# isarandi/metro-pose3d

Hardware: AMD Instinct MI355X
Metric: crops/sec (256x256, RN50 stride16) (higher is better)
Workload: dtype f16

## Files before the change

### include/metro_hip.h

```cpp
#ifndef METRO_HIP_H
#define METRO_HIP_H

#include <stddef.h>
#include <stdint.h>

#ifdef __cplusplus
extern "C" {
#endif

#define METRO_ABI_VERSION 8

typedef enum MetroStatus {
    METRO_OK = 0,
    METRO_ERR_INVALID_ARG = -1,
    METRO_ERR_UNSUPPORTED = -2,
    METRO_ERR_HIP = -3,
    METRO_ERR_STATE = -4,
    METRO_ERR_NONFINITE = -5
} MetroStatus;

typedef enum MetroPrecision { METRO_PREC_F16 = 0, METRO_PREC_F32 = 1, METRO_PREC_F64 = 2, METRO_PREC_F32M = 3 } MetroPrecision;

typedef enum MetroDType { METRO_F16 = 0, METRO_F32 = 1, METRO_F64 = 2 } MetroDType;

// ... 92 lines not shown
    int32_t h_out, w_out, c_out;
    int32_t kh, kw, stride, dilation;
    int32_t pad_top, pad_left;
    int32_t has_prologue;
    int32_t relu;
    int32_t has_residual;
    int32_t res_h, res_w;
    int32_t res_stride, res_offset;
    int32_t out_dtype;
    int32_t in_dtype;
} MetroConvDesc;

int  metro_conv_f16(const MetroConvDesc* d, const void* d_in, const void* d_w, const float* d_bias,
                    const void* d_pro_scale, const void* d_pro_shift, const void* d_residual,
                    void* d_out, void* stream);
int  metro_conv_f16_pair(const MetroConvDesc* d, const void* d_in, const void* d_w, const float* d_bias,
                         const void* d_pro_scale, const void* d_pro_shift, void* d_out, int32_t split,
                         void* d_out2, void* stream);
int  metro_conv_f16_next(const MetroConvDesc* d, const void* d_in, const void* d_w, const float* d_bias,
                         const void* d_residual, void* d_out, const void* d_w2, const float* d_bias2,
                         const void* d_scale2, const void* d_shift2, void* d_out2, int32_t c2, void* stream);
int  metro_conv_f16_conv1_conv2(const MetroConvDesc* d, const void* d_x, const void* d_w1, const float* d_bias1, const void* d_pro_scale,
                                const void* d_pro_shift, const void* d_w2, const float* d_bias2, void* d_out, void* stream);
int  metro_conv_f16_next_proj(const MetroConvDesc* d, const void* d_in, const void* d_w, const float* d_bias, const void* d_x,
                              const void* d_w_sc, const float* d_bias_sc, const void* d_pro_scale, const void* d_pro_shift, void* d_out,
                              const void* d_w2, const float* d_bias2, const void* d_scale2, const void* d_shift2, void* d_out2,
                              int32_t c2, void* stream);
int  metro_conv_f16_next_rebuild(const MetroConvDesc* d, const void* d_in, const void* d_w, const float* d_bias, const void* d_x,
                                 const void* d_w_sc, const float* d_bias_sc, const void* d_pro_scale, const void* d_pro_shift,
                                 const void* d_t2_prev, const void* d_w3_prev, const float* d_bias3_prev, void* d_out, void* d_out_sub,
                                 int32_t sub_off, const void* d_w2, const float* d_bias2, const void* d_scale2, const void* d_shift2,
                                 void* d_out2, int32_t c2, void* stream);
int  metro_conv_b1_form(int32_t classic);
int  metro_conv_f16_gemm4w(const MetroConvDesc* d, const void* d_in, const void* d_w, const float* d_bias,
                           const void* d_pro_scale, const void* d_pro_shift, const void* d_residual, void* d_out,
                           int32_t split, void* d_out2, void* stream);
int  metro_stem_pool_f16(const void* d_prepped, const void* d_w, const float* d_bias, void* d_out, int32_t n,
                         int32_t side, void* stream);
int  metro_stem_pool_f32in(const float* d_images, const void* d_w, const float* d_bias, void* d_out, int32_t n,
                           int32_t side, void* stream);
int  metro_stem_pool_u8in(const uint8_t* d_images, const void* d_w, const float* d_bias, void* d_out, int32_t n,
                          int32_t side, void* stream);
int  metro_conv_f64acc(const MetroConvDesc* d, const void* d_in, const double* d_w,
                       const double* d_bias, const double* d_pro_scale,
                       const double* d_pro_shift, const void* d_residual, void* d_out,
                       void* stream);

int  metro_conv_f32m(const MetroConvDesc* d, const void* d_in, const float* d_w, const float* d_bias, const float* d_pro_scale,
                     const float* d_pro_shift, const void* d_residual, void* d_out, void* stream);

int  metro_prep_input_f16(const float* d_images, int32_t n, int32_t side, void* d_out, void* stream);
int  metro_images_u8_to_f32(const uint8_t* d_in, int64_t count, float* d_out, void* stream);

int  metro_warp_crop_u8(const uint8_t* d_image, int32_t h, int32_t w, int32_t row_stride,
                        const float* d_homographies, int32_t n, int32_t side, float* d_out, void* stream);

#define METRO_MAX_FRAMES 64
#define METRO_WARP_HOMOGRAPHY 0
#define METRO_WARP_DISTORTED 1
typedef struct MetroFrame {
    const uint8_t* data;
    int32_t h, w, row_stride;
    int32_t reserved;
} MetroFrame;
typedef struct MetroCropWarp {
    int32_t frame;
// ... 217 lines not shown
```

### metro_pose3d_amd/_lib.py

```python
from __future__ import annotations

import ctypes as C
import os

HERE = os.path.dirname(os.path.abspath(__file__))
LIB_PATH = os.environ.get('METRO_HIP_LIB') or os.path.join(HERE, 'libmetro_hip.so')

METRO_MAX_JOINTS = 64
ABI_VERSION = 8
METRO_PREC_F16, METRO_PREC_F32, METRO_PREC_F64, METRO_PREC_F32M = 0, 1, 2, 3
METRO_F16, METRO_F32, METRO_F64 = 0, 1, 2
PARAM_CONV_W, PARAM_BIAS, PARAM_PRO_SCALE, PARAM_PRO_SHIFT = 0, 1, 2, 3
LAYER_PREP, LAYER_CONV, LAYER_POOL, LAYER_SOFTARGMAX = 0, 1, 2, 3
FUSED_CONV1_IN_FRONT, FUSED_PROJECTION_SHORTCUT = 1, 2
FUSED_OUT_ON_CHIP, FUSED_REBUILT_SHORTCUT, FUSED_COMPACT_SHORTCUT = 4, 8, 16


class MetroSpec(C.Structure):
    _fields_ = [('arch', C.c_int32), ('stride', C.c_int32), ('n_joints_head', C.c_int32),
                ('depth', C.c_int32), ('centered_stride', C.c_int32), ('proc_side', C.c_int32),
                ('box_size_mm', C.c_float), ('base_width', C.c_int32), ('precision', C.c_int32),
                ('n_joints_out', C.c_int32), ('permutation', C.c_int32 * METRO_MAX_JOINTS)]


# ... 91 lines not shown
class MetroView(C.Structure):
    _fields_ = [('cos_roll', C.c_double), ('sin_roll', C.c_double), ('zoom', C.c_double), ('flip', C.c_int32),
                ('reserved', C.c_int32)]


_P = C.c_void_p
SIGNATURES = {
    'metro_plan_create': (C.c_int, [C.POINTER(MetroSpec), C.c_int32, C.POINTER(_P)]),
    'metro_plan_destroy': (C.c_int, [_P]),
    'metro_plan_workspace_bytes': (C.c_int64, [_P]),
    'metro_plan_param_bytes': (C.c_int64, [_P]),
    'metro_plan_num_params': (C.c_int32, [_P]),
    'metro_plan_param_info': (C.c_int, [_P, C.c_int32, C.POINTER(MetroParamInfo)]),
    'metro_plan_num_layers': (C.c_int32, [_P]),
    'metro_plan_layer_info': (C.c_int, [_P, C.c_int32, C.POINTER(MetroLayerInfo)]),
    'metro_plan_flops_per_image': (C.c_double, [_P]),
    'metro_plan_bind_params': (C.c_int, [_P, _P]),
    'metro_plan_layer_kernel': (C.c_int, [_P, C.c_int32, C.c_int32, C.c_char_p, C.c_int32]),
    'metro_kernel_notes': (C.c_int, [C.c_int32]),
    'metro_last_kernel_id': (C.c_char_p, []),
    'metro_plan_set_graph_max_batch': (C.c_int, [_P, C.c_int32]),
    'metro_forward': (C.c_int, [_P, _P, C.c_int32, _P, _P, _P]),
    'metro_forward_coords01': (C.c_int, [_P, _P, C.c_int32, _P, _P, _P, _P]),
    'metro_forward_u8': (C.c_int, [_P, _P, C.c_int32, _P, _P, _P, _P]),
    'metro_forward_status': (C.c_int, [_P, _P, C.c_int32, _P, C.POINTER(C.c_int32)]),
    'metro_plan_status_offset': (C.c_int64, [_P]),
    'metro_forward_upto': (C.c_int, [_P, _P, C.c_int32, _P, _P, _P, C.c_int32]),
    'metro_forward_timed': (C.c_int, [_P, _P, C.c_int32, _P, _P, _P, C.POINTER(C.c_float)]),
    'metro_conv_f16': (C.c_int, [C.POINTER(MetroConvDesc), _P, _P, _P, _P, _P, _P, _P, _P]),
    'metro_conv_f32m': (C.c_int, [C.POINTER(MetroConvDesc), _P, _P, _P, _P, _P, _P, _P, _P]),
    'metro_conv_f64acc': (C.c_int, [C.POINTER(MetroConvDesc), _P, _P, _P, _P, _P, _P, _P, _P]),
    'metro_conv_f16_pair': (C.c_int, [C.POINTER(MetroConvDesc), _P, _P, _P, _P, _P, _P, C.c_int32, _P, _P]),
    'metro_conv_b1_form': (C.c_int, [C.c_int32]),
    'metro_conv_f16_gemm4w': (C.c_int, [C.POINTER(MetroConvDesc), _P, _P, _P, _P, _P, _P, _P, C.c_int32, _P, _P]),
    'metro_conv_f16_conv1_conv2': (C.c_int, [C.POINTER(MetroConvDesc), _P, _P, _P, _P, _P, _P, _P, _P, _P]),
    'metro_conv_f16_next_proj': (C.c_int, [C.POINTER(MetroConvDesc)] + [_P] * 14 + [C.c_int32, _P]),
    'metro_conv_f16_next_rebuild': (C.c_int, [C.POINTER(MetroConvDesc)] + [_P] * 13 + [C.c_int32] + [_P] * 5 + [C.c_int32, _P]),
    'metro_conv_f16_next': (C.c_int, [C.POINTER(MetroConvDesc), _P, _P, _P, _P, _P, _P, _P, _P, _P, _P, C.c_int32, _P]),
    'metro_stem_pool_f16': (C.c_int, [_P, _P, _P, _P, C.c_int32, C.c_int32, _P]),
    'metro_stem_pool_f32in': (C.c_int, [_P, _P, _P, _P, C.c_int32, C.c_int32, _P]),
    'metro_stem_pool_u8in': (C.c_int, [_P, _P, _P, _P, C.c_int32, C.c_int32, _P]),
    'metro_prep_input_f16': (C.c_int, [_P, C.c_int32, C.c_int32, _P, _P]),
    'metro_images_u8_to_f32': (C.c_int, [_P, C.c_int64, _P, _P]),
    'metro_warp_crop_u8': (C.c_int, [_P, C.c_int32, C.c_int32, C.c_int32, _P, C.c_int32, C.c_int32, _P, _P]),
    'metro_warp_crops_frames_u8': (C.c_int, [C.POINTER(MetroFrame), C.c_int32, _P, C.c_int32, C.c_int32, _P, _P]),
    'metro_warp_crops_frames_planes': (C.c_int, [C.POINTER(MetroFramePlanes), C.c_int32, _P, C.c_int32, C.c_int32, _P,
                                                 _P]),
    'metro_warp_crops_frames_u8_to_u8': (C.c_int, [C.POINTER(MetroFrame), C.c_int32, _P, C.c_int32, C.c_int32, _P, _P]),
    'metro_warp_crops_frames_planes_to_u8': (C.c_int, [C.POINTER(MetroFramePlanes), C.c_int32, _P, C.c_int32, C.c_int32, _P,
                                                       _P]),
    'metro_eval_metrics': (C.c_int, [_P, _P, _P, C.c_int32, C.c_int32, C.c_float, _P, _P, _P, _P]),
    'metro_maxpool3x3s2_zeropad': (C.c_int, [_P, _P, C.c_int32, C.c_int32, C.c_int32, C.c_int32,
                                             C.c_int32, _P]),
    'metro_softargmax_scratch_bytes': (C.c_int64, [C.c_int32, C.c_int32, C.c_int32]),
    'metro_softargmax01': (C.c_int, [_P, C.c_int32, C.POINTER(MetroSpec), C.c_int32, _P, _P, _P]),
    'metro_backproject_bone_lengths': (C.c_int, [_P, _P, _P, C.c_int32, _P, C.c_int32, C.c_int32, C.POINTER(MetroSpec),
                                                 C.c_int32, C.c_int32, _P, _P, _P]),
    'metro_backproject_root_depth': (C.c_int, [_P, _P, _P, C.c_int32, C.POINTER(MetroSpec), C.c_int32, C.c_int32, _P, _P]),
    'metro_to_orig_cam': (C.c_int, [_P, _P, _P, _P, C.c_int32, C.c_int32, _P]),
    'metro_place_poses': (C.c_int, [_P, _P, _P, C.c_int32, C.POINTER(MetroSpec), C.c_int32, _P, C.c_int32, _P, _P, C.c_int32,
                                    _P, C.c_int32, _P, _P, _P, _P]),
    'metro_expand_views': (C.c_int, [_P, C.c_int32, C.POINTER(MetroView), C.c_int32, C.c_int32, _P, _P, _P]),
    'metro_look_at_boxes': (C.c_int, [_P, _P, C.c_int32, C.c_int32, _P, C.c_int32, C.c_int32, _P, _P, _P]),
    'metro_merge_views': (C.c_int, [_P, _P, _P, _P, _P, C.c_int32, C.c_int32, C.c_int32, _P, _P, _P, _P, _P]),
    'metro_heatmap_to_25d': (C.c_int, [_P, C.c_int32, C.POINTER(MetroSpec), _P, _P]),
    'metro_head_f16_scratch_bytes': (C.c_int64, [C.c_int32, C.c_int32, C.c_int32]),
# ... 98 lines not shown
```

### metro_pose3d_amd/csrc/conv3x3_c64.hip

```cpp
#ifndef METRO_WT_STORES
#define METRO_WT_STORES 1
#endif
#include "metro_common.h"
#include "gfx950_prims.h"

namespace metro {

namespace c64 {
constexpr int C = 64, TN = 128, NW = 8, NT = 512;
constexpr int W_BYTES = 9 * C * 128;
constexpr int SLAB_ROWS = 256;
constexpr int SLAB_BYTES = SLAB_ROWS * 128;
constexpr int SI = SLAB_BYTES / 1024 / NW;
constexpr int WI = W_BYTES / 1024 / NW;
constexpr int W_OFF = 0;
constexpr int SLAB_OFF = W_BYTES;
constexpr int ZERO_OFF = SLAB_OFF + 2 * SLAB_BYTES;
constexpr int OUT_OFF = ZERO_OFF + 256;
constexpr int OUT_ROW = C * 2 + 16;
constexpr int LDS_BYTES = OUT_OFF + TN * OUT_ROW;
constexpr int STORES = TN * (C / 8) / NT;
static_assert(LDS_BYTES <= 160 * 1024 && ZERO_OFF % 256 == 0, "LDS budget / zero-area alignment");
}

struct C64Args {
    const half_t* in;
    const half_t* w;
    const float* bias;
    half_t* out;
    int m_total, h, w_map, relu, n_tiles, tiles_per_block;
    const half_t* w1;
    const float* bias1;
    const half_t* pro_scale;
    const half_t* pro_shift;
    half_t* t1_dump;
};

template <bool PRE1>
__global__ __launch_bounds__(c64::NT) void conv3x3_c64_kernel(C64Args a) {
    using namespace c64;
    extern __shared__ __attribute__((aligned(16))) char smem[];
    const int tid = threadIdx.x;
    const int lane = tid & 63;
    const int wave = __builtin_amdgcn_readfirstlane(tid >> 6);
    const int wm = wave >> 2, wn = wave & 3;
    const int frag_row = lane & 31, frag_half = lane >> 5;
    const int t_begin = blockIdx.x * a.tiles_per_block;
    int t_end = t_begin + a.tiles_per_block;
    if (t_end > a.n_tiles) t_end = a.n_tiles;
    if (t_begin >= t_end) return;
    const half_t* zero = reinterpret_cast<const half_t*>(g_zero_page);
    const unsigned smem_base = lds_offset_of(smem);
    const int halo = a.w_map;
    const int hw = a.h * a.w_map;

    if (tid < 16) reinterpret_cast<uint4*>(smem + ZERO_OFF)[tid] = make_uint4(0, 0, 0, 0);

    const int lrow = lane >> 3, lch = lane & 7;
#pragma unroll
    for (int i = 0; i < WI; ++i) {
        const int grp = i * NW + wave;
        const int tap = grp >> 3, row = (grp & 7) * 8 + lrow;
        const half_t* src = a.w + (size_t)row * (9 * C) + tap * C + ((lch ^ swz<64>(row)) * 8);
        dma16(src, __builtin_amdgcn_readfirstlane(smem_base + W_OFF + grp * 1024));
    }
    auto issue_slab = [&](int tile, int buf) {
        const int m0 = tile * TN;
#pragma unroll
        for (int i = 0; i < SI; ++i) {
            const int srow = (i * NW + wave) * 8 + lrow;
            const int g = m0 - halo + srow;
            const bool ok = g >= 0 && g < a.m_total && srow < TN + 2 * halo;
            const half_t* src = ok ? a.in + (size_t)g * C + ((lch ^ swz<64>(srow)) * 8) : zero;
            dma16(src, __builtin_amdgcn_readfirstlane(smem_base + SLAB_OFF + buf * SLAB_BYTES + (i * NW + wave) * 1024));
        }
    };
    issue_slab(t_begin, 0);

    const int arow = wm * 32 + frag_row;
    const int a_base = W_OFF + arow * 128 + ((frag_half ^ swz<64>(arow)) << 4);
    float bias_v[4][4];
#pragma unroll
    for (int q = 0; q < 4; ++q) {
        const floatx4 bv = *reinterpret_cast<const floatx4*>(a.bias + wm * 32 + 8 * q + 4 * frag_half);
#pragma unroll
        for (int e = 0; e < 4; ++e) bias_v[q][e] = bv[e];
    }
    half8_t w1f[2][4], ps1[4], pb1[4];
    float bias1_v[2][4][4];
    if constexpr (PRE1) {
#pragma unroll
        for (int i = 0; i < 2; ++i) {
#pragma unroll
            for (int kk = 0; kk < 4; ++kk)
                w1f[i][kk] = *reinterpret_cast<const half8_t*>(a.w1 + (size_t)(i * 32 + frag_row) * C + kk * 16 + frag_half * 8);
#pragma unroll
            for (int q = 0; q < 4; ++q) {
                const floatx4 bv = *reinterpret_cast<const floatx4*>(a.bias1 + i * 32 + 8 * q + 4 * frag_half);
#pragma unroll
                for (int e = 0; e < 4; ++e) bias1_v[i][q][e] = bv[e];
            }
        }
#pragma unroll
        for (int kk = 0; kk < 4; ++kk) {
            ps1[kk] = *reinterpret_cast<const half8_t*>(a.pro_scale + kk * 16 + frag_half * 8);
            pb1[kk] = *reinterpret_cast<const half8_t*>(a.pro_shift + kk * 16 + frag_half * 8);
        }
    }
    wait_vm_and_barrier<0>();

    for (int t = t_begin; t < t_end; ++t) {
        const int buf = (t - t_begin) & 1;
        if (t != t_begin) {
            asm volatile("s_waitcnt vmcnt(%0)\n\ts_barrier" ::"n"(STORES) : "memory");
        }
        if (t + 1 < t_end) issue_slab(t + 1, buf ^ 1);

        if constexpr (PRE1) {
            char* sp = smem + SLAB_OFF + buf * SLAB_BYTES;
            const int srow = wave * 32 + frag_row;
            const int r_base = srow * 128 + ((frag_half ^ swz<64>(srow)) << 4);
            floatx16 a1[2];
#pragma unroll
            for (int e = 0; e < 16; ++e) { a1[0][e] = 0.f; a1[1][e] = 0.f; }
#pragma unroll
            for (int kk = 0; kk < 4; ++kk) {
                half8_t bf = *reinterpret_cast<const half8_t*>(sp + (r_base ^ (kk << 5)));
                bf = relu(bf * ps1[kk] + pb1[kk]);
                a1[0] = __builtin_amdgcn_mfma_f32_32x32x16_f16(w1f[0][kk], bf, a1[0], 0, 0, 0);
                a1[1] = __builtin_amdgcn_mfma_f32_32x32x16_f16(w1f[1][kk], bf, a1[1], 0, 0, 0);
            }
#pragma unroll
            for (int i = 0; i < 2; ++i)
#pragma unroll
                for (int q = 0; q < 4; ++q) {
                    half4_t hv;
#pragma unroll
                    for (int e = 0; e < 4; ++e) hv[e] = (half_t)relu(a1[i][4 * q + e] + bias1_v[i][q][e]);
                    *reinterpret_cast<half4_t*>(sp + srow * 128 + ((((4 * i + q) ^ swz<64>(srow)) << 4) | (frag_half << 3))) = hv;
                    if (a.t1_dump != nullptr && srow >= halo && srow < halo + TN)
                        *reinterpret_cast<half4_t*>(a.t1_dump + (size_t)(t * TN + srow - halo) * C + i * 32 + 8 * q + 4 * frag_half) = hv;
                }
            wait_lgkm_and_barrier();
        }
        const int m0 = t * TN;
        const int tl = wn * 32 + frag_row;
        const int rem = (m0 + tl) % hw;
        const int py = rem / a.w_map, px = rem - py * a.w_map;
        floatx16 acc;
#pragma unroll
        for (int e = 0; e < 16; ++e) acc[e] = 0.f;
        const int sl = SLAB_OFF + buf * SLAB_BYTES;
#pragma unroll
        for (int tap = 0; tap < 9; ++tap) {
            const int dr = tap / 3 - 1, ds = tap % 3 - 1;
            const bool ok = (unsigned)(py + dr) < (unsigned)a.h && (unsigned)(px + ds) < (unsigned)a.w_map;
            const int srow = halo + tl + dr * a.w_map + ds;
            const int b_base = ok ? sl + srow * 128 + ((frag_half ^ swz<64>(srow)) << 4) : ZERO_OFF;
#pragma unroll
            for (int kk = 0; kk < 4; ++kk) {
                const half8_t af = *reinterpret_cast<const half8_t*>(smem + tap * 8192 + (a_base ^ (kk << 5)));
                const half8_t bf = *reinterpret_cast<const half8_t*>(smem + (b_base ^ (kk << 5)));
                acc = __builtin_amdgcn_mfma_f32_32x32x16_f16(af, bf, acc, 0, 0, 0);
            }
        }
        char* ol = smem + OUT_OFF;
#pragma unroll
        for (int q = 0; q < 4; ++q) {
            half4_t hv;
#pragma unroll
            for (int e = 0; e < 4; ++e) {
                float v = acc[4 * q + e] + bias_v[q][e];
                if (a.relu) v = relu(v);
                hv[e] = (half_t)v;
            }
            *reinterpret_cast<half4_t*>(ol + tl * OUT_ROW + (wm * 32 + 8 * q + 4 * frag_half) * 2) = hv;
        }
        wait_lgkm_and_barrier();
#pragma unroll
        for (int r = 0; r < STORES; ++r) {
            const int idx = tid + r * NT;
            const int prow = idx >> 3, ch = idx & 7;
            const uint4 v = *reinterpret_cast<const uint4*>(ol + prow * OUT_ROW + ch * 16);
            store_out16(a.out + (size_t)(m0 + prow) * C + ch * 8, v);
        }
    }
}

bool conv3x3_c64_supported(const MetroConvDesc& d) {
    static const int enabled = tuning_knob("METRO_CONV_C64", 1);
    if (!enabled) return false;
    if (!(d.kh == 3 && d.kw == 3 && d.stride == 1 && d.dilation == 1 && d.pad_top == 1 && d.pad_left == 1 &&
          d.h_in == d.h_out && d.w_in == d.w_out && d.c_in == 64 && d.c_out == 64 && d.in_pix_stride == 64 &&
          !d.has_prologue && !d.has_residual && d.in_dtype == METRO_F16 && d.out_dtype == METRO_F16))
        return false;
    const long m = (long)d.n * d.h_out * d.w_out;
    return d.w_out <= 64 && c64::TN % d.w_out == 0 && (d.h_out * d.w_out) % c64::TN == 0 && m >= 4 * c64::TN;
}

int launch_conv3x3_c64(const MetroConvDesc& d, const void* in, const void* w, const float* bias, void* out, hipStream_t stream,
                       const ConvPre1* pre1) {
    if (!conv3x3_c64_supported(d)) { set_error("conv3x3_c64: unsupported layer"); return METRO_ERR_UNSUPPORTED; }
    const bool p1 = pre1 != nullptr && pre1->w1 != nullptr;
    if (note_kernel(p1 ? "conv3x3_c64<pre1>" : "conv3x3_c64")) return METRO_OK;
    C64Args a;
    a.in = static_cast<const half_t*>(in); a.w = static_cast<const half_t*>(w); a.bias = bias; a.out = static_cast<half_t*>(out);
    a.m_total = d.n * d.h_out * d.w_out; a.h = d.h_out; a.w_map = d.w_out; a.relu = d.relu;
    a.n_tiles = a.m_total / c64::TN;
    a.w1 = p1 ? static_cast<const half_t*>(pre1->w1) : nullptr; a.bias1 = p1 ? pre1->bias1 : nullptr;
    a.pro_scale = p1 ? static_cast<const half_t*>(pre1->pro_scale) : nullptr;
    a.pro_shift = p1 ? static_cast<const half_t*>(pre1->pro_shift) : nullptr;
    a.t1_dump = p1 ? static_cast<half_t*>(pre1->t1_dump) : nullptr;
    auto kern = p1 ? conv3x3_c64_kernel<true> : conv3x3_c64_kernel<false>;
    static PerDeviceInt cap[2];
    int grid_cap = 0;
    if (const int st = ensure_dyn_lds_and_grid_cap(reinterpret_cast<const void*>(kern), c64::NT, c64::LDS_BYTES, cap[p1 ? 1 : 0],
                                                   "conv3x3_c64", 1, &grid_cap))
        return st;
    a.tiles_per_block = (a.n_tiles + grid_cap - 1) / grid_cap;
    const int grid = (a.n_tiles + a.tiles_per_block - 1) / a.tiles_per_block;
    hipLaunchKernelGGL(kern, dim3(grid), dim3(c64::NT), c64::LDS_BYTES, stream, a);
    return launch_status("conv3x3_c64");
}

}
```

### metro_pose3d_amd/csrc/entries.cpp

```cpp
#include <cmath>
#include <cstring>

#include "metro_common.h"

namespace metro {

static thread_local char g_err[512] = "";

void set_error(const char* fmt, ...) {
    va_list ap;
    va_start(ap, fmt);
    vsnprintf(g_err, sizeof(g_err), fmt, ap);
    va_end(ap);
}
const char* get_error() { return g_err; }

static thread_local KernelNotes g_notes = {0, ""};
KernelNotes& kernel_notes() { return g_notes; }
bool note_kernel(const char* fmt, ...) {
    if (g_notes.mode == 0) return false;
    const size_t cap = sizeof(g_notes.ids) - 5;
    const size_t used = strlen(g_notes.ids);
    if (used >= 4 && strcmp(g_notes.ids + used - 4, " ...") == 0) return g_notes.mode == 2;
    char one[512];
// ... 65 lines not shown
                           static_cast<hipStream_t>(stream));
}

int metro_conv_f16_pair(const MetroConvDesc* d, const void* d_in, const void* d_w, const float* d_bias,
                        const void* d_pro_scale, const void* d_pro_shift, void* d_out, int32_t split,
                        void* d_out2, void* stream) {
    int st = validate_conv_desc(d);
    if (st) return st;
    METRO_CHECK_ARG(d_in && d_w && d_bias && d_out && d_out2 && d_pro_scale && d_pro_shift, "conv_f16_pair: NULL tensor pointer");
    ConvFused f;
    f.form = ConvForm::Pair;
    f.pair = {split, d->c_out - split, 1, d_out2};
    METRO_CHECK_ARG(conv_form_supported(*d, f), "conv_f16_pair: fp16 1x1 stride-1 convolution with prologue, without residual / ReLU on the "
                    "first output, c_in %% 64; split %d of c_out %d (split %% 256, rest %% 8)", split, d->c_out);
    return launch_conv_f16_dma(*d, d_in, d_w, d_bias, d_pro_scale, d_pro_shift, nullptr, d_out, static_cast<hipStream_t>(stream), f);
}

int metro_conv_f16_next(const MetroConvDesc* d, const void* d_in, const void* d_w, const float* d_bias,
                        const void* d_residual, void* d_out, const void* d_w2, const float* d_bias2,
                        const void* d_scale2, const void* d_shift2, void* d_out2, int32_t c2, void* stream) {
    int st = validate_conv_desc(d);
    if (st) return st;
    METRO_CHECK_ARG(d_in && d_w && d_bias && d_out && d_w2 && d_bias2 && d_scale2 && d_shift2 && d_out2,
                    "conv_f16_next: NULL tensor pointer");
    METRO_CHECK_ARG(!d->has_residual || d_residual, "conv_f16_next: residual tensor missing");
    ConvFused f;
    f.form = ConvForm::Next;
    f.next = {d_w2, d_bias2, d_scale2, d_shift2, d_out2, c2};
    METRO_CHECK_ARG(conv_form_supported(*d, f),
                    "conv_f16_next: built for 1x1 stride-1 64 -> 256 with c2 = 64 (block1) and 128 -> 512 with c2 = 128 (block2), fp16");
    return launch_conv_f16_dma(*d, d_in, d_w, d_bias, nullptr, nullptr, d_residual, d_out, static_cast<hipStream_t>(stream), f);
}

int metro_conv_f16_conv1_conv2(const MetroConvDesc* d, const void* d_x, const void* d_w1, const float* d_bias1, const void* d_pro_scale,
                               const void* d_pro_shift, const void* d_w2, const float* d_bias2, void* d_out, void* stream) {
    int st = validate_conv_desc(d);
    if (st) return st;
    METRO_CHECK_ARG(d_x && d_w1 && d_bias1 && d_pro_scale && d_pro_shift && d_w2 && d_bias2 && d_out, "conv_f16_conv1_conv2: NULL tensor pointer");
    METRO_CHECK_ARG(conv3x3_c64_supported(*d), "conv_f16_conv1_conv2: built for 3x3 stride-1 SAME 64 -> 64 on maps of <= 64 columns that tile into "
                    "128-pixel row pairs (block1 of the 256-pixel nets)");
    ConvPre1 p1;
    p1.w1 = d_w1; p1.bias1 = d_bias1; p1.pro_scale = d_pro_scale; p1.pro_shift = d_pro_shift;
    return launch_conv3x3_c64(*d, d_x, d_w2, d_bias2, d_out, static_cast<hipStream_t>(stream), &p1);
}

int metro_conv_f16_next_proj(const MetroConvDesc* d, const void* d_in, const void* d_w, const float* d_bias, const void* d_x,
                             const void* d_w_sc, const float* d_bias_sc, const void* d_pro_scale, const void* d_pro_shift, void* d_out,
                             const void* d_w2, const float* d_bias2, const void* d_scale2, const void* d_shift2, void* d_out2,
                             int32_t c2, void* stream) {
    int st = validate_conv_desc(d);
    if (st) return st;
    METRO_CHECK_ARG(d_in && d_w && d_bias && d_x && d_w_sc && d_bias_sc && d_pro_scale && d_pro_shift && d_w2 && d_bias2 &&
                        d_scale2 && d_shift2 && d_out2, "conv_f16_next_proj: NULL tensor pointer");
    ConvFused f;
    f.form = ConvForm::NextProj;
    f.next = {d_w2, d_bias2, d_scale2, d_shift2, d_out2, c2};
    f.psc = {d_x, d_w_sc, d_bias_sc, d_pro_scale, d_pro_shift};
    f.rb.out_mode = d_out == nullptr ? 1 : 0;
    METRO_CHECK_ARG(conv_form_supported(*d, f), "conv_f16_next_proj: built for 1x1 stride-1 64 -> 256 without prologue / residual, "
                    "c2 = 64 (block1/unit_1), fp16");
    return launch_conv_f16_dma(*d, d_in, d_w, d_bias, nullptr, nullptr, nullptr, d_out, static_cast<hipStream_t>(stream), f);
}

int metro_conv_f16_next_rebuild(const MetroConvDesc* d, const void* d_in, const void* d_w, const float* d_bias, const void* d_x,
                                const void* d_w_sc, const float* d_bias_sc, const void* d_pro_scale, const void* d_pro_shift,
                                const void* d_t2_prev, const void* d_w3_prev, const float* d_bias3_prev, void* d_out, void* d_out_sub,
                                int32_t sub_off, const void* d_w2, const float* d_bias2, const void* d_scale2, const void* d_shift2,
                                void* d_out2, int32_t c2, void* stream) {
    int st = validate_conv_desc(d);
    if (st) return st;
    METRO_CHECK_ARG(d_in && d_w && d_bias && d_x && d_w_sc && d_bias_sc && d_pro_scale && d_pro_shift && d_t2_prev && d_w3_prev && d_bias3_prev &&
                        d_w2 && d_bias2 && d_scale2 && d_shift2 && d_out2, "conv_f16_next_rebuild: NULL tensor pointer");
    METRO_CHECK_ARG((d_out != nullptr) != (d_out_sub != nullptr), "conv_f16_next_rebuild: exactly one of d_out (the whole sum) and d_out_sub (its "
                    "sub-sampled compact copy) must be given");
    METRO_CHECK_ARG(sub_off == 0 || sub_off == 1, "conv_f16_next_rebuild: sub_off %d must be 0 or 1", sub_off);
    ConvFused f;
    f.form = ConvForm::NextRebuild;
    f.next = {d_w2, d_bias2, d_scale2, d_shift2, d_out2, c2};
    f.psc = {d_x, d_w_sc, d_bias_sc, d_pro_scale, d_pro_shift};
    ConvRebuild& rb = f.rb;
    rb.t2_prev = d_t2_prev; rb.w3_prev = d_w3_prev; rb.bias3_prev = d_bias3_prev;
    if (d_out_sub != nullptr) {
        rb.out_mode = 2; rb.out_sub = d_out_sub; rb.sub_off = sub_off;
        rb.h_sub = (d->h_out - sub_off + 1) / 2; rb.w_sub = (d->w_out - sub_off + 1) / 2;
    }
    METRO_CHECK_ARG(conv_form_supported(*d, f), "conv_f16_next_rebuild: built for 1x1 stride-1 64 -> 256 without prologue / residual on maps "
                    "whose width is a power of two >= 16 and whose pixel count is a multiple of 64, c2 = 64 (block1/unit_2), fp16");
    return launch_conv_f16_dma(*d, d_in, d_w, d_bias, nullptr, nullptr, nullptr, d_out, static_cast<hipStream_t>(stream), f);
}

int metro_conv_b1_form(int32_t classic) {
    METRO_CHECK_ARG(classic == 0 || classic == 1, "metro_conv_b1_form: 0 (default dispatch) or 1 (classic single-role kernel)");
    conv_b1_set_form(classic);
    return METRO_OK;
}

int metro_conv_f16_gemm4w(const MetroConvDesc* d, const void* d_in, const void* d_w, const float* d_bias,
                          const void* d_pro_scale, const void* d_pro_shift, const void* d_residual, void* d_out,
                          int32_t split, void* d_out2, void* stream) {
    int st = validate_conv_desc(d);
    if (st) return st;
    METRO_CHECK_ARG(d_in && d_w && d_bias && d_out, "conv_f16_gemm4w: NULL tensor pointer");
    METRO_CHECK_ARG(!d->has_prologue || (d_pro_scale && d_pro_shift), "conv_f16_gemm4w: prologue tensors missing");
    METRO_CHECK_ARG(!d->has_residual || d_residual, "conv_f16_gemm4w: residual tensor missing");
    METRO_CHECK_ARG(split >= 0 && split < d->c_out && (split == 0 || d_out2), "conv_f16_gemm4w: bad split %d / missing second output", split);
    ConvSplit sp;
    sp.split = split; sp.c_out2 = d->c_out - split; sp.relu2 = 1; sp.out2 = d_out2;
    return launch_conv_gemm4w(*d, d_in, d_w, d_bias, d_pro_scale, d_pro_shift, d_residual, d_out,
                              static_cast<hipStream_t>(stream), split > 0 ? &sp : nullptr);
}

int metro_stem_pool_f16(const void* d_prepped, const void* d_w, const float* d_bias, void* d_out, int32_t n,
                        int32_t side, void* stream) {
    METRO_CHECK_ARG(d_prepped && d_w && d_bias && d_out, "stem_pool_f16: NULL tensor pointer");
    METRO_CHECK_ARG(n > 0, "stem_pool_f16: n = %d", n);
    METRO_CHECK_ARG(stem_pool_f16_supported(side, 64), "stem_pool_f16: side %d must be a multiple of 32 (and METRO_STEM_POOL != 0)", side);
    return launch_stem_pool_f16(d_prepped, d_w, d_bias, d_out, n, side, static_cast<hipStream_t>(stream));
}

int metro_stem_pool_f32in(const float* d_images, const void* d_w, const float* d_bias, void* d_out, int32_t n,
                          int32_t side, void* stream) {
    METRO_CHECK_ARG(d_images && d_w && d_bias && d_out, "stem_pool_f32in: NULL tensor pointer");
    METRO_CHECK_ARG(n > 0, "stem_pool_f32in: n = %d", n);
    METRO_CHECK_ARG(stem_pool_f32in_supported(side, 64), "stem_pool_f32in: side %d must be a multiple of 32 (and METRO_STEM_POOL / METRO_STEM_RAW != 0)", side);
    return launch_stem_pool_f32in(d_images, d_w, d_bias, d_out, n, side, static_cast<hipStream_t>(stream));
}
// ... 588 lines not shown
```

### metro_pose3d_amd/csrc/metro_common.h

```cpp
#pragma once
#include <hip/hip_runtime.h>
#include <cstdarg>
#include <cstdint>
#include <cstdio>
#include <cstdlib>

#include "../../include/metro_hip.h"

namespace metro {

void set_error(const char* fmt, ...);
const char* get_error();

#define METRO_CHECK_ARG(cond, ...)                  \
    do {                                            \
        if (!(cond)) {                              \
            ::metro::set_error(__VA_ARGS__);        \
            return METRO_ERR_INVALID_ARG;           \
        }                                           \
    } while (0)

#define METRO_HIP_CHECK(expr)                                                              \
    do {                                                                                   \
        hipError_t _e = (expr);                                                            \
// ... 219 lines not shown
                    const void* pro_scale, const void* pro_shift, const void* residual, void* out,
                    hipStream_t stream);
bool conv_f16_dma_supported(const MetroConvDesc& d);
int launch_conv_f16_dma(const MetroConvDesc& d, const void* in, const void* w, const float* bias,
                        const void* pro_scale, const void* pro_shift, const void* residual, void* out,
                        hipStream_t stream, const ConvFused& f = ConvFused{});
bool conv_form_supported(const MetroConvDesc& d, const ConvFused& f);
bool conv_f16_fuse2_supported(const MetroConvDesc& d, int c2);
bool conv_gemm4w_shape_ok(const MetroConvDesc& d, const ConvSplit* split);
bool conv_gemm4w_supported(const MetroConvDesc& d, const ConvSplit* split);
int launch_conv_gemm4w(const MetroConvDesc& d, const void* in, const void* w, const float* bias, const void* pro_scale,
                       const void* pro_shift, const void* residual, void* out, hipStream_t stream, const ConvSplit* split);
bool conv_pw64_supported(const MetroConvDesc& d, const ConvFused& f);
int launch_conv_pw64(const MetroConvDesc& d, const void* in, const void* w, const float* bias, const void* pro_scale,
                     const void* pro_shift, const void* residual, void* out, hipStream_t stream, const ConvFused& f);
bool conv_b1_chain_preferred();
void conv_b1_set_form(int classic);
bool classic_forms_forced();
bool conv_pws_supported(const MetroConvDesc& d);
int launch_conv_pws(const MetroConvDesc& d, const void* in, const void* w, const float* bias, const void* res, void* out, hipStream_t stream);
int launch_conv_b1_chain(const MetroConvDesc& d, const void* in, const void* w, const float* bias, void* out, hipStream_t stream,
                         const ConvFused& f);
bool stem_pool_f16_supported(int side, int base_width);
int launch_stem_pool_f16(const void* prepped, const void* w, const float* bias, void* out, int n, int side,
                         hipStream_t stream);
bool stem_pool_f32in_supported(int side, int base_width);
int launch_stem_pool_f32in(const float* images, const void* w, const float* bias, void* out, int n, int side,
                           hipStream_t stream);
int launch_stem_pool_u8in(const unsigned char* images, const void* w, const float* bias, void* out, int n, int side,
                          hipStream_t stream);
bool conv3x3_c64_supported(const MetroConvDesc& d);
int launch_conv3x3_c64(const MetroConvDesc& d, const void* in, const void* w, const float* bias, void* out, hipStream_t stream,
                       const ConvPre1* pre1 = nullptr);
bool conv3x3_slab_supported(const MetroConvDesc& d);
int launch_conv3x3_slab(const MetroConvDesc& d, const void* in, const void* w, const float* bias, void* out,
                        hipStream_t stream);
int launch_conv_f64acc(const MetroConvDesc& d, const void* in, const double* w, const double* bias,
                       const double* pro_scale, const double* pro_shift, const void* residual,
                       void* out, hipStream_t stream);
int launch_conv_f32m(const MetroConvDesc& d, const void* in, const float* w, const float* bias, const float* pro_scale,
                     const float* pro_shift, const void* residual, void* out, hipStream_t stream);
int launch_prep_input_f16(const float* images, int n, int side, void* out, hipStream_t stream);
int launch_prep_input_u8_f16(const unsigned char* images, int n, int side, void* out, hipStream_t stream);
int launch_images_u8_to_f32(const unsigned char* in, long count, float* out, hipStream_t stream);
struct FrameTable { MetroFrame f[METRO_MAX_FRAMES]; };
template <typename OutT>
int launch_warp_crops_frames_u8(const FrameTable& frames, int n_frames, const MetroCropWarp* crops, int n, int side,
                                OutT* out, hipStream_t stream);
struct FramePlanesTable { MetroFramePlanes f[METRO_MAX_FRAMES]; };
template <typename OutT>
int launch_warp_crops_frames_planes(const FramePlanesTable& frames, int n_frames, const MetroCropWarp* crops, int n,
                                    int side, OutT* out, hipStream_t stream);
template <typename OutT>
int launch_warp_crop_u8(const unsigned char* img, int h, int w, int row_stride, const float* homs, OutT* out,
                        int n, int side, hipStream_t stream);
int launch_eval_metrics(const float* pred, const float* truth, const unsigned char* valid, int n, int nj,
                        float threshold, float* dist, float* dist_pa, double* sums, hipStream_t stream);
int launch_maxpool(const void* in, void* out, int n, int h_in, int w_in, int c, int dtype,
                   hipStream_t stream);

struct SoftArgmaxArgs {
    int n, side, depth, n_joints_head, n_joints_out;
    int lrc, half_off;
    float box_size_mm;
    int proc_side;
    int perm[METRO_MAX_JOINTS];
// ... 81 lines not shown
```

Measured before the change: 47140.

## Stream conv3x3 c64 input through a 3-segment ring to reuse halo rows

Replaces the per-tile double-buffered slab (each tile reloading its full halo window) with a three-segment ring buffer. Each new tile loads only one segment, and with the fused conv1 prologue only the new rows are recomputed instead of redoing the halo. Output staging is double-buffered so the global store of tile j-1 overlaps the MMA work of tile j. Row and column bounds checks become shift/mask precomputation, which assumes a power-of-two map width. Debug hooks for a grid cap and a t1 dump are also added.

Result: no change. 47320, median of 5 (+0.4%).

```diff
diff --git a/include/metro_hip.h b/include/metro_hip.h
--- a/include/metro_hip.h
+++ b/include/metro_hip.h
@@ -148,6 +148,8 @@
                                  int32_t sub_off, const void* d_w2, const float* d_bias2, const void* d_scale2, const void* d_shift2,
                                  void* d_out2, int32_t c2, void* stream);
 int  metro_conv_b1_form(int32_t classic);
+int  metro_conv_c64_grid_cap(int32_t cap);
+int  metro_conv_c64_t1_dump(void* d_t1);
 int  metro_conv_f16_gemm4w(const MetroConvDesc* d, const void* d_in, const void* d_w, const float* d_bias,
                            const void* d_pro_scale, const void* d_pro_shift, const void* d_residual, void* d_out,
                            int32_t split, void* d_out2, void* stream);
diff --git a/metro_pose3d_amd/_lib.py b/metro_pose3d_amd/_lib.py
--- a/metro_pose3d_amd/_lib.py
+++ b/metro_pose3d_amd/_lib.py
@@ -147,6 +147,8 @@
     'metro_conv_f64acc': (C.c_int, [C.POINTER(MetroConvDesc), _P, _P, _P, _P, _P, _P, _P, _P]),
     'metro_conv_f16_pair': (C.c_int, [C.POINTER(MetroConvDesc), _P, _P, _P, _P, _P, _P, C.c_int32, _P, _P]),
     'metro_conv_b1_form': (C.c_int, [C.c_int32]),
+    'metro_conv_c64_grid_cap': (C.c_int, [C.c_int32]),
+    'metro_conv_c64_t1_dump': (C.c_int, [_P]),
     'metro_conv_f16_gemm4w': (C.c_int, [C.POINTER(MetroConvDesc), _P, _P, _P, _P, _P, _P, _P, C.c_int32, _P, _P]),
     'metro_conv_f16_conv1_conv2': (C.c_int, [C.POINTER(MetroConvDesc), _P, _P, _P, _P, _P, _P, _P, _P, _P]),
     'metro_conv_f16_next_proj': (C.c_int, [C.POINTER(MetroConvDesc)] + [_P] * 14 + [C.c_int32, _P]),
diff --git a/metro_pose3d_amd/csrc/conv3x3_c64.hip b/metro_pose3d_amd/csrc/conv3x3_c64.hip
--- a/metro_pose3d_amd/csrc/conv3x3_c64.hip
+++ b/metro_pose3d_amd/csrc/conv3x3_c64.hip
@@ -9,18 +9,24 @@
 namespace c64 {
 constexpr int C = 64, TN = 128, NW = 8, NT = 512;
 constexpr int W_BYTES = 9 * C * 128;
-constexpr int SLAB_ROWS = 256;
-constexpr int SLAB_BYTES = SLAB_ROWS * 128;
-constexpr int SI = SLAB_BYTES / 1024 / NW;
+constexpr int HALO = 64;
+constexpr int SEG_BYTES = TN * 128;
+constexpr int RING_ROWS = 3 * TN;
+constexpr int RING_BYTES = RING_ROWS * 128;
+constexpr int SI0 = (TN + 2 * HALO) / 8 / NW;
+constexpr int SI = TN / 8 / NW;
 constexpr int WI = W_BYTES / 1024 / NW;
 constexpr int W_OFF = 0;
-constexpr int SLAB_OFF = W_BYTES;
-constexpr int ZERO_OFF = SLAB_OFF + 2 * SLAB_BYTES;
+constexpr int RING_OFF = W_BYTES;
+constexpr int ZERO_OFF = RING_OFF + RING_BYTES;
 constexpr int OUT_OFF = ZERO_OFF + 256;
 constexpr int OUT_ROW = C * 2 + 16;
-constexpr int LDS_BYTES = OUT_OFF + TN * OUT_ROW;
+constexpr int OUT_BYTES = TN * OUT_ROW;
+constexpr int LDS_BYTES = OUT_OFF + 2 * OUT_BYTES;
 constexpr int STORES = TN * (C / 8) / NT;
-static_assert(LDS_BYTES <= 160 * 1024 && ZERO_OFF % 256 == 0, "LDS budget / zero-area alignment");
+static_assert(LDS_BYTES == 73728 + 49152 + 256 + 2 * 18432 && LDS_BYTES <= 160 * 1024 && ZERO_OFF % 256 == 0,
+              "LDS budget / zero-area alignment");
+static_assert(TN + 2 * HALO == 2 * TN && RING_ROWS % 16 == 0 && TN % 16 == 0, "a window is two segments; the chunk swizzle has period 16 rows");
 }
 
 struct C64Args {
@@ -28,7 +34,7 @@
     const half_t* w;
     const float* bias;
     half_t* out;
-    int m_total, h, w_map, relu, n_tiles, tiles_per_block;
+    int m_total, h, w_map, w_shift, relu, n_tiles, tiles_per_block;
     const half_t* w1;
     const float* bias1;
     const half_t* pro_scale;
@@ -49,9 +55,11 @@
     int t_end = t_begin + a.tiles_per_block;
     if (t_end > a.n_tiles) t_end = a.n_tiles;
     if (t_begin >= t_end) return;
+    const int n_loc = t_end - t_begin;
+    const int m_begin = t_begin * TN;
+    const int g0 = m_begin - HALO;
     const half_t* zero = reinterpret_cast<const half_t*>(g_zero_page);
     const unsigned smem_base = lds_offset_of(smem);
-    const int halo = a.w_map;
     const int hw = a.h * a.w_map;
 
     if (tid < 16) reinterpret_cast<uint4*>(smem + ZERO_OFF)[tid] = make_uint4(0, 0, 0, 0);
@@ -64,18 +72,17 @@
         const half_t* src = a.w + (size_t)row * (9 * C) + tap * C + ((lch ^ swz<64>(row)) * 8);
         dma16(src, __builtin_amdgcn_readfirstlane(smem_base + W_OFF + grp * 1024));
     }
-    auto issue_slab = [&](int tile, int buf) {
-        const int m0 = tile * TN;
-#pragma unroll
-        for (int i = 0; i < SI; ++i) {
-            const int srow = (i * NW + wave) * 8 + lrow;
-            const int g = m0 - halo + srow;
-            const bool ok = g >= 0 && g < a.m_total && srow < TN + 2 * halo;
-            const half_t* src = ok ? a.in + (size_t)g * C + ((lch ^ swz<64>(srow)) * 8) : zero;
-            dma16(src, __builtin_amdgcn_readfirstlane(smem_base + SLAB_OFF + buf * SLAB_BYTES + (i * NW + wave) * 1024));
+    auto issue_rows = [&](auto n_instr, int u0, int seg) {
+#pragma unroll
+        for (int i = 0; i < decltype(n_instr)::value; ++i) {
+            const int row = (i * NW + wave) * 8 + lrow;
+            const int g = g0 + u0 + row;
+            const bool ok = g >= 0 && g < a.m_total;
+            const half_t* src = ok ? a.in + (size_t)g * C + ((lch ^ swz<64>(row)) * 8) : zero;
+            dma16(src, __builtin_amdgcn_readfirstlane(smem_base + RING_OFF + seg + (i * NW + wave) * 1024));
         }
     };
-    issue_slab(t_begin, 0);
+    issue_rows(std::integral_constant<int, SI0>{}, 0, 0);
 
     const int arow = wm * 32 + frag_row;
     const int a_base = W_OFF + arow * 128 + ((frag_half ^ swz<64>(arow)) << 4);
@@ -107,56 +114,101 @@
             pb1[kk] = *reinterpret_cast<const half8_t*>(a.pro_shift + kk * 16 + frag_half * 8);
         }
     }
+    auto conv1_rows = [&](int rrow, int u) {
+        char* rp = smem + RING_OFF;
+        const int r_base = rrow * 128 + ((frag_half ^ swz<64>(rrow)) << 4);
+        floatx16 a1[2];
+#pragma unroll
+        for (int e = 0; e < 16; ++e) { a1[0][e] = 0.f; a1[1][e] = 0.f; }
+#pragma unroll
+        for (int kk = 0; kk < 4; ++kk) {
+            half8_t bf = *reinterpret_cast<const half8_t*>(rp + (r_base ^ (kk << 5)));
+            bf = relu(bf * ps1[kk] + pb1[kk]);
+            a1[0] = __builtin_amdgcn_mfma_f32_32x32x16_f16(w1f[0][kk], bf, a1[0], 0, 0, 0);
+            a1[1] = __builtin_amdgcn_mfma_f32_32x32x16_f16(w1f[1][kk], bf, a1[1], 0, 0, 0);
+        }
+        const bool dump = a.t1_dump != nullptr && u >= HALO && u < HALO + n_loc * TN;
+#pragma unroll
+        for (int i = 0; i < 2; ++i)
+#pragma unroll
+            for (int q = 0; q < 4; ++q) {
+                half4_t hv;
+#pragma unroll
+                for (int e = 0; e < 4; ++e) hv[e] = (half_t)relu(a1[i][4 * q + e] + bias1_v[i][q][e]);
+                *reinterpret_cast<half4_t*>(rp + rrow * 128 + ((((4 * i + q) ^ swz<64>(rrow)) << 4) | (frag_half << 3))) = hv;
+                if (dump)
+                    *reinterpret_cast<half4_t*>(a.t1_dump + (size_t)(g0 + u) * C + i * 32 + 8 * q + 4 * frag_half) = hv;
+            }
+    };
+    auto store_tile = [&](int j) {
+        const char* ol = smem + OUT_OFF + (j & 1) * OUT_BYTES;
+        uint4 v[STORES];
+#pragma unroll
+        for (int r = 0; r < STORES; ++r) {
+            const int idx = tid + r * NT;
+            v[r] = *reinterpret_cast<const uint4*>(ol + (idx >> 3) * OUT_ROW + (idx & 7) * 16);
+        }
+#pragma unroll
+        for (int r = 0; r < STORES; ++r) {
+            const int idx = tid + r * NT;
+            store_out16(a.out + (size_t)(m_begin + j * TN + (idx >> 3)) * C + (idx & 7) * 8, v[r]);
+        }
+    };
+    const int tl = wn * 32 + frag_row;
+    const int px = tl & (a.w_map - 1), prow_t = tl >> a.w_shift;
+    const bool ok_l = px > 0, ok_r = px + 1 < a.w_map;
+    int tap_off[9];
+#pragma unroll
+    for (int tap = 0; tap < 9; ++tap) {
+        const int u = HALO + tl + (tap / 3 - 1) * a.w_map + (tap % 3 - 1);
+        tap_off[tap] = u * 128 + ((frag_half ^ swz<64>(u)) << 4);
+    }
+#pragma unroll
+    for (int q = 0; q < 4; ++q)
+#pragma unroll
+        for (int e = 0; e < 4; ++e) asm volatile("" : "+v"(bias_v[q][e]));
+    if constexpr (PRE1) {
+#pragma unroll
+        for (int kk = 0; kk < 4; ++kk) {
+            asm volatile("" : "+v"(w1f[0][kk]), "+v"(w1f[1][kk]), "+v"(ps1[kk]), "+v"(pb1[kk]));
+#pragma unroll
+            for (int e = 0; e < 4; ++e) asm volatile("" : "+v"(bias1_v[0][kk][e]), "+v"(bias1_v[1][kk][e]));
+        }
+    }
+    int rem = m_begin % hw;
+    int rb = 0;
     wait_vm_and_barrier<0>();
 
-    for (int t = t_begin; t < t_end; ++t) {
-        const int buf = (t - t_begin) & 1;
-        if (t != t_begin) {
-            asm volatile("s_waitcnt vmcnt(%0)\n\ts_barrier" ::"n"(STORES) : "memory");
-        }
-        if (t + 1 < t_end) issue_slab(t + 1, buf ^ 1);
+    for (int j = 0; j < n_loc; ++j) {
+        if (j == 1) wait_vm_and_barrier<0>();
+        else if (j > 1) asm volatile("s_waitcnt vmcnt(%0) lgkmcnt(0)\n\ts_barrier" ::"n"(STORES) : "memory");
+        const int seg1 = rb + SEG_BYTES < RING_BYTES ? rb + SEG_BYTES : 0;
+        const int seg2 = seg1 + SEG_BYTES < RING_BYTES ? seg1 + SEG_BYTES : 0;
+        if (j + 1 < n_loc) issue_rows(std::integral_constant<int, SI>{}, (j + 2) * TN, seg2);
+        if (PRE1 && j > 0) store_tile(j - 1);
 
         if constexpr (PRE1) {
-            char* sp = smem + SLAB_OFF + buf * SLAB_BYTES;
-            const int srow = wave * 32 + frag_row;
-            const int r_base = srow * 128 + ((frag_half ^ swz<64>(srow)) << 4);
-            floatx16 a1[2];
-#pragma unroll
-            for (int e = 0; e < 16; ++e) { a1[0][e] = 0.f; a1[1][e] = 0.f; }
-#pragma unroll
-            for (int kk = 0; kk < 4; ++kk) {
-                half8_t bf = *reinterpret_cast<const half8_t*>(sp + (r_base ^ (kk << 5)));
-                bf = relu(bf * ps1[kk] + pb1[kk]);
-                a1[0] = __builtin_amdgcn_mfma_f32_32x32x16_f16(w1f[0][kk], bf, a1[0], 0, 0, 0);
-                a1[1] = __builtin_amdgcn_mfma_f32_32x32x16_f16(w1f[1][kk], bf, a1[1], 0, 0, 0);
-            }
-#pragma unroll
-            for (int i = 0; i < 2; ++i)
-#pragma unroll
-                for (int q = 0; q < 4; ++q) {
-                    half4_t hv;
-#pragma unroll
-                    for (int e = 0; e < 4; ++e) hv[e] = (half_t)relu(a1[i][4 * q + e] + bias1_v[i][q][e]);
-                    *reinterpret_cast<half4_t*>(sp + srow * 128 + ((((4 * i + q) ^ swz<64>(srow)) << 4) | (frag_half << 3))) = hv;
-                    if (a.t1_dump != nullptr && srow >= halo && srow < halo + TN)
-                        *reinterpret_cast<half4_t*>(a.t1_dump + (size_t)(t * TN + srow - halo) * C + i * 32 + 8 * q + 4 * frag_half) = hv;
-                }
+            if (j == 0) {
+                conv1_rows(wave * 32 + frag_row, wave * 32 + frag_row);
+            } else if (wave < 4) {
+                const int row = wave * 32 + frag_row;
+                conv1_rows((seg1 >> 7) + row, (j + 1) * TN + row);
+            }
             wait_lgkm_and_barrier();
         }
-        const int m0 = t * TN;
-        const int tl = wn * 32 + frag_row;
-        const int rem = (m0 + tl) % hw;
-        const int py = rem / a.w_map, px = rem - py * a.w_map;
+        const int py = (rem >> a.w_shift) + prow_t;
+        const bool ok_u = py > 0, ok_d = py + 1 < a.h;
         floatx16 acc;
 #pragma unroll
         for (int e = 0; e < 16; ++e) acc[e] = 0.f;
-        const int sl = SLAB_OFF + buf * SLAB_BYTES;
+        if (!PRE1 && j > 0) store_tile(j - 1);
 #pragma unroll
         for (int tap = 0; tap < 9; ++tap) {
             const int dr = tap / 3 - 1, ds = tap % 3 - 1;
-            const bool ok = (unsigned)(py + dr) < (unsigned)a.h && (unsigned)(px + ds) < (unsigned)a.w_map;
-            const int srow = halo + tl + dr * a.w_map + ds;
-            const int b_base = ok ? sl + srow * 128 + ((frag_half ^ swz<64>(srow)) << 4) : ZERO_OFF;
+            const bool ok = (dr < 0 ? ok_u : dr > 0 ? ok_d : true) && (ds < 0 ? ok_l : ds > 0 ? ok_r : true);
+            int roff = tap_off[tap] + rb;
+            if (roff >= RING_BYTES) roff -= RING_BYTES;
+            const int b_base = ok ? RING_OFF + roff : ZERO_OFF;
 #pragma unroll
             for (int kk = 0; kk < 4; ++kk) {
                 const half8_t af = *reinterpret_cast<const half8_t*>(smem + tap * 8192 + (a_base ^ (kk << 5)));
@@ -164,7 +216,7 @@
                 acc = __builtin_amdgcn_mfma_f32_32x32x16_f16(af, bf, acc, 0, 0, 0);
             }
         }
-        char* ol = smem + OUT_OFF;
+        char* ol = smem + OUT_OFF + (j & 1) * OUT_BYTES;
 #pragma unroll
         for (int q = 0; q < 4; ++q) {
             half4_t hv;
@@ -176,16 +228,16 @@
             }
             *reinterpret_cast<half4_t*>(ol + tl * OUT_ROW + (wm * 32 + 8 * q + 4 * frag_half) * 2) = hv;
         }
-        wait_lgkm_and_barrier();
-#pragma unroll
-        for (int r = 0; r < STORES; ++r) {
-            const int idx = tid + r * NT;
-            const int prow = idx >> 3, ch = idx & 7;
-            const uint4 v = *reinterpret_cast<const uint4*>(ol + prow * OUT_ROW + ch * 16);
-            store_out16(a.out + (size_t)(m0 + prow) * C + ch * 8, v);
-        }
-    }
-}
+        rb = seg1;
+        rem += TN;
+        if (rem >= hw) rem = 0;
+    }
+    wait_lgkm_and_barrier();
+    store_tile(n_loc - 1);
+}
+
+static thread_local int g_c64_grid_cap = 0;
+void conv3x3_c64_set_grid_cap(int cap) { g_c64_grid_cap = cap; }
 
 bool conv3x3_c64_supported(const MetroConvDesc& d) {
     static const int enabled = tuning_knob("METRO_CONV_C64", 1);
@@ -207,6 +259,7 @@
     a.in = static_cast<const half_t*>(in); a.w = static_cast<const half_t*>(w); a.bias = bias; a.out = static_cast<half_t*>(out);
     a.m_total = d.n * d.h_out * d.w_out; a.h = d.h_out; a.w_map = d.w_out; a.relu = d.relu;
     a.n_tiles = a.m_total / c64::TN;
+    a.w_shift = __builtin_ctz((unsigned)d.w_out);
     a.w1 = p1 ? static_cast<const half_t*>(pre1->w1) : nullptr; a.bias1 = p1 ? pre1->bias1 : nullptr;
     a.pro_scale = p1 ? static_cast<const half_t*>(pre1->pro_scale) : nullptr;
     a.pro_shift = p1 ? static_cast<const half_t*>(pre1->pro_shift) : nullptr;
@@ -217,6 +270,7 @@
     if (const int st = ensure_dyn_lds_and_grid_cap(reinterpret_cast<const void*>(kern), c64::NT, c64::LDS_BYTES, cap[p1 ? 1 : 0],
                                                    "conv3x3_c64", 1, &grid_cap))
         return st;
+    if (g_c64_grid_cap > 0 && g_c64_grid_cap < grid_cap) grid_cap = g_c64_grid_cap;
     a.tiles_per_block = (a.n_tiles + grid_cap - 1) / grid_cap;
     const int grid = (a.n_tiles + a.tiles_per_block - 1) / a.tiles_per_block;
     hipLaunchKernelGGL(kern, dim3(grid), dim3(c64::NT), c64::LDS_BYTES, stream, a);
diff --git a/metro_pose3d_amd/csrc/entries.cpp b/metro_pose3d_amd/csrc/entries.cpp
--- a/metro_pose3d_amd/csrc/entries.cpp
+++ b/metro_pose3d_amd/csrc/entries.cpp
@@ -121,6 +121,8 @@
     return launch_conv_f16_dma(*d, d_in, d_w, d_bias, nullptr, nullptr, d_residual, d_out, static_cast<hipStream_t>(stream), f);
 }
 
+static thread_local void* g_c64_t1_dump = nullptr;
+
 int metro_conv_f16_conv1_conv2(const MetroConvDesc* d, const void* d_x, const void* d_w1, const float* d_bias1, const void* d_pro_scale,
                                const void* d_pro_shift, const void* d_w2, const float* d_bias2, void* d_out, void* stream) {
     int st = validate_conv_desc(d);
@@ -130,6 +132,7 @@
                     "128-pixel row pairs (block1 of the 256-pixel nets)");
     ConvPre1 p1;
     p1.w1 = d_w1; p1.bias1 = d_bias1; p1.pro_scale = d_pro_scale; p1.pro_shift = d_pro_shift;
+    p1.t1_dump = g_c64_t1_dump;
     return launch_conv3x3_c64(*d, d_x, d_w2, d_bias2, d_out, static_cast<hipStream_t>(stream), &p1);
 }
 
@@ -181,6 +184,17 @@
 int metro_conv_b1_form(int32_t classic) {
     METRO_CHECK_ARG(classic == 0 || classic == 1, "metro_conv_b1_form: 0 (default dispatch) or 1 (classic single-role kernel)");
     conv_b1_set_form(classic);
+    return METRO_OK;
+}
+
+int metro_conv_c64_grid_cap(int32_t cap) {
+    METRO_CHECK_ARG(cap >= 0, "metro_conv_c64_grid_cap: %d must be 0 (default grid) or an upper bound on the grid", cap);
+    conv3x3_c64_set_grid_cap(cap);
+    return METRO_OK;
+}
+
+int metro_conv_c64_t1_dump(void* d_t1) {
+    g_c64_t1_dump = d_t1;
     return METRO_OK;
 }
 
diff --git a/metro_pose3d_amd/csrc/metro_common.h b/metro_pose3d_amd/csrc/metro_common.h
--- a/metro_pose3d_amd/csrc/metro_common.h
+++ b/metro_pose3d_amd/csrc/metro_common.h
@@ -275,6 +275,7 @@
 bool conv3x3_c64_supported(const MetroConvDesc& d);
 int launch_conv3x3_c64(const MetroConvDesc& d, const void* in, const void* w, const float* bias, void* out, hipStream_t stream,
                        const ConvPre1* pre1 = nullptr);
+void conv3x3_c64_set_grid_cap(int cap);
 bool conv3x3_slab_supported(const MetroConvDesc& d);
 int launch_conv3x3_slab(const MetroConvDesc& d, const void* in, const void* w, const float* bias, void* out,
                         hipStream_t stream);
```
